# FangjinhuaWang/PatchmatchNet

Measured on AMD Instinct MI355X. Metric: depth-maps/sec at 1600x1200 N=5 src views, higher is better.
Workload: dtype f32

## Files before the change

### include/pmn_hip.h

```cpp
#ifndef PMN_HIP_H
#define PMN_HIP_H

#include <stdint.h>

#ifdef __cplusplus
extern "C" {
#endif

#define PMN_ABI_VERSION 25
#define PMN_MLP_FLOATS 340
#define PMN_MAX_DEPTH 64
#define PMN_MAX_NEIGHBORS 17
#define PMN_MAX_FUSE_SRC 32
#define PMN_TSDF_MAX_VIEWS 16
#define PMN_TSDF_MARK_SPAN 8
#define PMN_RASTER_MAX_DIM 16384
#define PMN_RASTER_MAX_BOX 64
#define PMN_SPLAT_MAX_RADIUS 32

#define PMN_OK 0
#define PMN_ERR_ARG (-1)
#define PMN_ERR_SHAPE (-2)
#define PMN_ERR_LAUNCH (-3)

// ... 36 lines not shown
               int W, int cin, int cout, int K, int stride, int pad, int dil, int relu, int in_nchw, int out_nchw,
               int up_h, int up_w, void *stream);

int pmn_fpn_tail(const float *x, const float *up, const float *w_in, const float *b_in, const float *w_out, float *out,
                 int N, int H, int W, int cin, int cmid, int cout, void *stream);

int pmn_conv2d_mfma(const float *in, const float *weights, const float *shift, float *out, float *out_b, int N, int H, int W,
                    int cin, int cout, int ca, int K, int stride, int pad, int dil, int relu, int planar, void *stream);


int pmn_conv2d_f16s(const float *in, const void *weights, const float *shift, float *out, int N, int H, int W, int cin, int cout,
                    int k, int stride, int relu, void *stream);

int pmn_conv2d_f16s_pair(const float *in, const void *weights_a, const float *shift_a, const void *weights_b, const float *shift_b,
                         float *out, int N, int H, int W, int channels, int relu, void *stream);

int pmn_offset_heads_f16s(const float *in, const void *weights, const float *shift, float *out_a, float *out_b, int N, int H, int W,
                          int cin, int cout, int ca, int dil, void *stream);

int pmn_fpn_level(const float *x, const float *u, const float *w, const float *b, float *out_a, float *out_b, int N, int H,
                  int W, int cin, int cout, int ca, void *stream);

int pmn_deconv3x3s2(const float *in, const float *weights, const float *shift, float *out, int N, int Hi, int Wi, int cin,
                    int cout, int relu, void *stream);

int pmn_refine_front(const float *img, const float *t2, const float *w0, const float *s0, const float *wd, const float *sd,
                     float *x16, int B, int H, int W, void *stream);
int pmn_refine_tail(const float *x16, const float *w3, const float *s3, const float *wr, const float *dnorm,
                    const float *depth_min, const float *depth_max, float *out, int B, int H, int W, void *stream);

int pmn_refine_fused(const float *img, const float *t2, const float *w0, const float *s0, const float *wd, const float *sd,
                     const void *w3a, const float *s3, const float *wr, const float *dnorm, const float *depth_min,
                     const float *depth_max, float *out, int B, int H, int W, void *stream);

int pmn_stage_projections(const float *intrinsics, const float *extrinsics, int B, int V, int nstages, float scale0,
                          float *rel, void *stream);

int pmn_stem(const float *img, const float *w0, const float *s0, const float *w1, const float *s1, float *out, int N, int H,
             int W, void *stream);

int pmn_stem_f16s(const float *img, const float *w0, const float *s0, const void *w1a, const float *s1, float *out, int N, int H,
                  int W, void *stream);

int pmn_stem_f16s_views(const float *const *img_table, int views, const float *w0, const float *s0, const void *w1a,
                        const float *s1, float *out, int B, int H, int W, void *stream);

int pmn_differentiable_warping(const float *src_nchw, const float *rel_proj, const float *depth, int B, int C,
                               int D, int h, int w, int hs, int ws, float *warped, void *stream);

int pmn_fuse_view(const float *maps, long long slot_stride, int ref_slot, const int *src_slots_host,
                  const int *src_hw_host, int n_src, const float *mats, int H, int W, float geo_pixel_thres, float geo_depth_thres, int geo_mask_thres,
                  float photo_thres, unsigned char *masks, float *xyz, double *depth_avg, int *geo_sum, void *stream);

int pmn_fuse_view_merged(const float *maps, long long slot_stride, int ref_slot, const int *src_slots_host,
                         const int *src_hw_host, int n_src, const float *mats, int H, int W, float geo_pixel_thres,
                         float geo_depth_thres, int geo_mask_thres, float photo_thres, unsigned char *masks, float *xyz,
                         double *depth_avg, int *geo_sum, unsigned char *claimed, long long claim_stride, unsigned char *emit,
                         void *stream);

int pmn_pack_points(const unsigned char *final_mask, const float *xyz, const void *image_hwc, int image_is_float, int H, int W,
                    unsigned char *records, long long capacity_points, long long *cursor, int *view_count, long long *scratch,
                    void *stream);

int pmn_pack_points_normals(const unsigned char *final_mask, const float *xyz, const float *normals_chw, const float *rotation,
                            int rotation_stride, const void *image_hwc, int image_is_float, int H, int W, unsigned char *records,
                            long long capacity_points, long long *cursor, int *view_count, long long *scratch, void *stream);
// ... 156 lines not shown
```

### patchmatchnet_amd/_lib.py

```python
from __future__ import annotations

import ctypes
import os
import subprocess
from typing import Optional

_CSRC = os.path.join(os.path.dirname(os.path.abspath(__file__)), "csrc")
LIB_PATH = os.path.join(_CSRC, "libpmn_hip.so")
ABI_VERSION = 25
MLP_FLOATS = 340
MAX_DEPTH = 64
MAX_NEIGHBORS = 17
MAX_FUSE_SRC = 32
TSDF_MAX_VIEWS = 16
TSDF_MARK_SPAN = 8
RASTER_MAX_DIM = 16384
RASTER_MAX_BOX = 64
SPLAT_MAX_RADIUS = 32
ICP_SUMS = 17
ICP_LIMBS = 5
ICP_BLOCK_POINTS = 256
VOXEL_LONG_RUN = 256
VOXEL_MAX_CHANNELS = 8
CROP_MAX_VERTICES = 4096
MESH_PLACE_LONG_RUN = 256
MESH_SIMPLIFY_MAX_FACES = 715827882
MESH_SMOOTH_LONG_ROW = 256
MESH_SMOOTH_MAX_STEPS = 65536
NORMAL_SWEEPS = 6
NORMAL_MAX_VIEWPOINTS = 4096

_fp = ctypes.c_void_p
_ip = ctypes.c_void_p
_hp = ctypes.c_void_p
_i = ctypes.c_int
_f = ctypes.c_float
_s = ctypes.c_void_p

SIGNATURES = {
    "pmn_abi_version": [],
    "pmn_error_string": [_i],
    "pmn_nchw_to_nhwc": [_fp, _fp, _i, _i, _i, _i, _s],
    "pmn_feature_weight": [_fp, _fp, _hp, _fp, _i, _i, _i, _i, _i, _i, _fp, _s],
    "pmn_init_hypotheses": [_fp, _fp, _i, _fp, _fp, _i, _f, _fp, _hp, _i, _i, _i, _i, _fp, _fp, _s],
    "pmn_warp_correlate": [_fp, _fp, _fp, _fp, _fp, _i, _fp, _fp, _i, _i, _i, _i, _i, _i, _i, _i, _i, _fp, _fp, _ip,
                           _fp, _s],
    "pmn_warp_correlate_views": [_fp, _fp, _fp, _fp, _fp, _i, _fp, _fp, _i, _i, _i, _i, _i, _i, _i, _i, _i, _fp, _fp, _ip,
                                 _fp, _s],
    "pmn_aggregate_regress": [_fp, _fp, _fp, _fp, _fp, _hp, _i, _f, _i, _i, _i, _i, _i, _fp, _fp, _s],
    "pmn_confidence": [_fp, _i, _i, _i, _i, _i, _i, _fp, _ip, _s],
    "pmn_conv2d": [_fp, _fp, _fp, _fp, _fp] + [_i] * 14 + [_s],
    "pmn_fpn_tail": [_fp] * 6 + [_i] * 6 + [_s],
    "pmn_fpn_level": [_fp] * 6 + [_i] * 6 + [_s],
    "pmn_conv2d_f16s": [_fp] * 4 + [_i] * 8 + [_s],
    "pmn_offset_heads_f16s": [_fp] * 5 + [_i] * 7 + [_s],
    "pmn_conv2d_f16s_pair": [_fp] * 6 + [_i] * 5 + [_s],
    "pmn_refine_front": [_fp] * 7 + [_i] * 3 + [_s],
    "pmn_refine_tail": [_fp] * 8 + [_i] * 3 + [_s],
    "pmn_refine_fused": [_fp] * 13 + [_i] * 3 + [_s],
    "pmn_conv2d_mfma": [_fp] * 5 + [_i] * 12 + [_s],
    "pmn_deconv3x3s2": [_fp] * 4 + [_i] * 6 + [_s],
    "pmn_stage_projections": [_fp, _fp, _i, _i, _i, _f, _fp, _s],
    "pmn_stem": [_fp] * 6 + [_i] * 3 + [_s],
    "pmn_stem_f16s": [_fp] * 6 + [_i] * 3 + [_s],
    "pmn_stem_f16s_views": [_fp, _i] + [_fp] * 5 + [_i] * 3 + [_s],
    "pmn_differentiable_warping": [_fp, _fp, _fp, _i, _i, _i, _i, _i, _i, _i, _fp, _s],
    "pmn_fuse_view": [_fp, ctypes.c_longlong, _i, _hp, _hp, _i, _fp, _i, _i, _f, _f, _i, _f, _fp, _fp, _fp, _ip, _s],
    "pmn_fuse_view_merged": [_fp, ctypes.c_longlong, _i, _hp, _hp, _i, _fp, _i, _i, _f, _f, _i, _f, _fp, _fp, _fp, _ip, _fp,
                             ctypes.c_longlong, _fp, _s],
    "pmn_pack_points": [_fp, _fp, _fp, _i, _i, _i, _fp, ctypes.c_longlong, _fp, _ip, _fp, _s],
    "pmn_pack_points_normals": [_fp, _fp, _fp, _fp, _i, _fp, _i, _i, _i, _fp, ctypes.c_longlong, _fp, _ip, _fp, _s],
    "pmn_depth_normals": [_fp, _i, _i, _hp, _i, _f, _fp, _s],
    "pmn_normalize_depth": [_fp, _fp, _fp, _i, _i, _fp, _s],
    "pmn_check_f16_domain": [_fp, ctypes.c_longlong, _ip, _s],
    "pmn_plan_create": [ctypes.POINTER(ctypes.c_void_p)],
    "pmn_plan_begin": [_hp],
    "pmn_plan_end": [_hp],
    "pmn_plan_count": [_hp],
    "pmn_plan_kernel_name": [_hp, _i],
    "pmn_plan_launch": [_hp, _s],
    "pmn_plan_destroy": [_hp],
    "pmn_plan_fork": [_hp],
    "pmn_plan_switch": [_hp, _i],
    "pmn_plan_join": [_hp],
    "pmn_plan_entry_branch": [_hp, _i],
    "pmn_plan_launch_part": [_hp, _i, _s],
    "pmn_view_scores": [_fp] * 6 + [_i, _i, ctypes.c_longlong, ctypes.c_longlong] + [ctypes.c_double] * 3 + [_fp, _s],
    "pmn_depth_metrics": [_fp, _fp, _hp, _hp, _hp, _i, _hp, _i, _i, _i, _i, _fp, ctypes.c_longlong, _fp, _s],
    "pmn_nn_distance": [_fp, _ip, ctypes.c_longlong, _hp, ctypes.c_double, _hp, _fp, _ip, ctypes.c_longlong, ctypes.c_double, _fp, _ip,
                        _s],
    "pmn_reduce_round": [_fp, _ip, ctypes.c_longlong, _hp, ctypes.c_double, _hp, ctypes.c_double, _ip, _ip, _ip, _s],
    "pmn_tsdf_integrate": [_fp] * 4 + [_hp, _hp, _f, _f, _fp, ctypes.c_longlong] + [_hp] * 5 + [_i, _s],
# ... 101 lines not shown
```

### patchmatchnet_amd/csrc/misc.hip

```cpp
#include <cstring>

#include "pmn_common.hpp"

extern "C" int pmn_abi_version(void) { return PMN_ABI_VERSION; }

extern "C" const char* pmn_error_string(int code) {
    switch (code) {
        case PMN_OK: return "ok";
        case PMN_ERR_ARG: return "invalid argument (null pointer or size out of range)";
        case PMN_ERR_SHAPE: return "unsupported shape (channels/groups/neighbours/hypotheses)";
        case PMN_ERR_LAUNCH: return "HIP launch failed";
        default: return "unknown error";
    }
}

__global__ __launch_bounds__(PMN_BLOCK) void nchw_to_nhwc_kernel(const float* __restrict__ in, float* __restrict__ out,
                                                                int C, int hw) {
    extern __shared__ float tile[];
    const int b = blockIdx.y, p0 = blockIdx.x * 64, tid = threadIdx.x;
    for (int idx = tid; idx < C * 64; idx += PMN_BLOCK) {
        const int c = idx >> 6, i = idx & 63;
        tile[c * 65 + i] = (p0 + i < hw) ? in[((size_t)b * C + c) * hw + p0 + i] : 0.0f;
    }
    __syncthreads();
// ... 175 lines not shown
            for (int k = 0; k < 4; ++k) acc = acc + P[1][r * 4 + k] * (float)A[k][4 + c];
            o[r * 4 + c] = acc;
        }
}

extern "C" int pmn_stage_projections(const float* intrinsics, const float* extrinsics, int B, int V, int nstages,
                                     float scale0, float* rel, void* stream) {
    if (!intrinsics || !extrinsics || !rel || B < 1 || V < 2 || nstages < 1) return PMN_ERR_ARG;
    const int total = nstages * B * (V - 1);
    PMN_LAUNCH(stage_projections_kernel, dim3((total + 63) / 64), dim3(64), 0, (hipStream_t)stream, intrinsics,
                       extrinsics, B, V, nstages, scale0, rel);
    PMN_CHECK_LAUNCH();
    return PMN_OK;
}

__global__ __launch_bounds__(PMN_BLOCK) void normalize_depth_kernel(const float* __restrict__ depth, const float* __restrict__ depth_min,
                                                                    const float* __restrict__ depth_max, int n, float* __restrict__ out) {
#pragma clang fp contract(off)
    const int b = blockIdx.y, i = blockIdx.x * PMN_BLOCK + threadIdx.x;
    if (i >= n) return;
    const float lo = depth_min[b], span = depth_max[b] - lo;
    out[(size_t)b * n + i] = (depth[(size_t)b * n + i] - lo) / span;
}

extern "C" int pmn_normalize_depth(const float* depth, const float* depth_min, const float* depth_max, int B, int n, float* out,
                                   void* stream) {
    if (!depth || !depth_min || !depth_max || !out || B < 1 || n < 1) return PMN_ERR_ARG;
    PMN_LAUNCH(normalize_depth_kernel, dim3((n + PMN_BLOCK - 1) / PMN_BLOCK, B), dim3(PMN_BLOCK), 0, (hipStream_t)stream, depth,
               depth_min, depth_max, n, out);
    PMN_CHECK_LAUNCH();
    return PMN_OK;
}

__global__ __launch_bounds__(PMN_BLOCK) void check_f16_domain_kernel(const float* __restrict__ x, long long n, int* __restrict__ flag) {
    bool bad = false;
    for (long long i = blockIdx.x * (long long)PMN_BLOCK + threadIdx.x; i < n; i += (long long)gridDim.x * PMN_BLOCK) {
        const float v = fabsf(x[i]);
        bad |= !(v < 65504.0f);
    }
    if (__any(bad) && (threadIdx.x & 63) == 0) atomicOr(flag, 1);
}

extern "C" int pmn_check_f16_domain(const float* x, long long n, int* flag, void* stream) {
    if (!x || !flag || n < 1) return PMN_ERR_ARG;
    const long long blocks = (n + PMN_BLOCK - 1) / PMN_BLOCK;
    PMN_LAUNCH(check_f16_domain_kernel, dim3((unsigned)(blocks < 4096 ? blocks : 4096)), dim3(PMN_BLOCK), 0, (hipStream_t)stream, x, n, flag);
    PMN_CHECK_LAUNCH();
    return PMN_OK;
}
```

### patchmatchnet_amd/csrc/refine.hip

```cpp
#include "conv_common.hpp"

typedef const float __attribute__((address_space(4))) cfloat;

__global__ __launch_bounds__(PMN_BLOCK) void refine_front_kernel(const float* __restrict__ img, const float* __restrict__ t2,
                                                                 const float* __restrict__ w0, const float* __restrict__ s0,
                                                                 const float* __restrict__ wd, const float* __restrict__ sd,
                                                                 float* __restrict__ x16, int B, int H, int W) {
    constexpr int TW = 16, TH = 16, IW = 18, IWP = 19, TP = 9, TPP = 12;
    __shared__ float xin[3 * IW * IWP];
    __shared__ float4 tp4[TP * TP * TPP / 4];
    float* tp = reinterpret_cast<float*>(tp4);
    const cfloat* cw0 = (const cfloat*)w0;
    const cfloat* cs0 = (const cfloat*)s0;
    const cfloat* cwd = (const cfloat*)wd;
    const cfloat* csd = (const cfloat*)sd;
    const int tid = threadIdx.x, wave = __builtin_amdgcn_readfirstlane(tid >> 6), lane = tid & 63;
    const int tiles_x = (W + TW - 1) / TW, tiles_y = (H + TH - 1) / TH;
    const int bt = pmn_xcd_tile(blockIdx.x, B * tiles_x * tiles_y);
    const int n = bt / (tiles_x * tiles_y), tr = bt - n * tiles_x * tiles_y;
    const int oy0 = (tr / tiles_x) * TH, ox0 = (tr % tiles_x) * TW;
    const int Hi = H / 2, Wi = W / 2, iy0 = oy0 / 2, ix0 = ox0 / 2;

    {
        constexpr int NL = (3 * IW * IW + PMN_BLOCK - 1) / PMN_BLOCK;
// ... 158 lines not shown
#pragma unroll
    for (int ky = 0; ky < 3; ++ky)
#pragma unroll
        for (int kx = 0; kx < 3; ++kx) {
            const float* mp = mid + (ty + ky) * MRP + (tx + kx) * MP;
            const float4 a = *reinterpret_cast<const float4*>(mp), b = *reinterpret_cast<const float4*>(mp + 4);
            const cfloat* wq = cwr + (ky * 3 + kx) * 8;
            res = fmaf(a.x, wq[0], res); res = fmaf(a.y, wq[1], res); res = fmaf(a.z, wq[2], res); res = fmaf(a.w, wq[3], res);
            res = fmaf(b.x, wq[4], res); res = fmaf(b.y, wq[5], res); res = fmaf(b.z, wq[6], res); res = fmaf(b.w, wq[7], res);
        }
    const int oy = oy0 + ty, ox = ox0 + tx;
    if (oy >= H || ox >= W) return;
    {
#pragma clang fp contract(off)
        const float lo = dmin[n], span = dmax[n] - lo;
        const float d = dnorm[((size_t)n * (H / 2) + (oy >> 1)) * (W / 2) + (ox >> 1)] + res;
        out[((size_t)n * H + oy) * W + ox] = d * span + lo;
    }
}

extern "C" int pmn_refine_tail(const float* x16, const float* w3, const float* s3, const float* wr, const float* dnorm,
                               const float* depth_min, const float* depth_max, float* out, int B, int H, int W, void* stream) {
    if (!x16 || !w3 || !s3 || !wr || !dnorm || !depth_min || !depth_max || !out || B < 1 || H < 2 || W < 2 || (H & 1) || (W & 1))
        return PMN_ERR_ARG;
    const size_t lds = (size_t)(20 * 424 + 18 * 256) * sizeof(float);
    if (pmn_raise_dynamic_lds(reinterpret_cast<const void*>(refine_tail_kernel), lds) != PMN_OK) return PMN_ERR_LAUNCH;
    const int blocks = B * ((W + 15) / 16) * ((H + 15) / 16);
    PMN_LAUNCH(refine_tail_kernel, dim3(blocks), dim3(PMN_BLOCK), lds, (hipStream_t)stream, x16, w3, s3, wr, dnorm,
                       depth_min, depth_max, out, B, H, W);
    PMN_CHECK_LAUNCH();
    return PMN_OK;
}

template <bool VEC4>
__global__ __launch_bounds__(PMN_BLOCK, 3) void refine_fused_kernel(
    const float* __restrict__ img, const float* __restrict__ t2, const float* __restrict__ w0, const float* __restrict__ s0,
    const float* __restrict__ wd, const float* __restrict__ sd, const f16x8* __restrict__ w3A, const float* __restrict__ s3,
    const float* __restrict__ wr, const float* __restrict__ dnorm, const float* __restrict__ dmin, const float* __restrict__ dmax,
    float* __restrict__ out, int B, int H, int W) {
    constexpr int TW = 16, TH = 16;
    constexpr int IR = 22, IC = 24;
    constexpr int TP = 11, TPP = 12;
    constexpr int XW = 20, XROWP = 26, XPIX = 16;
    constexpr int XPLANE = XW * XROWP * XPIX;
    constexpr int MW = 18, MP = 12, MRP = 256;
    extern __shared__ float4 rf_lds4[];
    _Float16* xh = reinterpret_cast<_Float16*>(rf_lds4);
    float* region = reinterpret_cast<float*>(xh + 2 * XPLANE);
    float* xin = region;
    float* tp = region + 3 * IR * IC;
    float* mid = region;
    const cfloat* cw0 = (const cfloat*)w0;
    const cfloat* cs0 = (const cfloat*)s0;
    const cfloat* cwd = (const cfloat*)wd;
    const cfloat* csd = (const cfloat*)sd;
    const cfloat* cwr = (const cfloat*)wr;
    const int tid = threadIdx.x, wave = __builtin_amdgcn_readfirstlane(tid >> 6), lane = tid & 63, li = lane & 15, kb = lane >> 4;
    const int tiles_x = (W + TW - 1) / TW, tiles_y = (H + TH - 1) / TH;
    const int bt = pmn_xcd_tile(blockIdx.x, B * tiles_x * tiles_y);
    const int n = bt / (tiles_x * tiles_y), tr = bt - n * tiles_x * tiles_y;
    const int oy0 = (tr / tiles_x) * TH, ox0 = (tr % tiles_x) * TW;
    const int Hi = H / 2, Wi = W / 2, iy0 = oy0 / 2 - 1, ix0 = ox0 / 2 - 1;

    {
        float4 u = make_float4(0.f, 0.f, 0.f, 0.f);
        const int upix = tid >> 1, uq = tid & 1;
        const int ur = upix / TP, uc = upix - ur * TP;
        if (upix < TP * TP) {
            const int gy = iy0 + ur, gx = ix0 + uc;
            if ((unsigned)gy < (unsigned)Hi && (unsigned)gx < (unsigned)Wi)
                u = *reinterpret_cast<const float4*>(t2 + (((size_t)n * Hi + gy) * Wi + gx) * 8 + 4 * uq);
        }
        if constexpr (VEC4) {
            float4 v[3];
            const int j = tid & 7, gx = ox0 - 4 + 4 * j;
#pragma unroll
            for (int k = 0; k < 3; ++k) {
                const int R = (tid >> 3) + 32 * k;
                const int c = (R >= IR) + (R >= 2 * IR), r = R - IR * c, gy = oy0 - 3 + r;
                v[k] = make_float4(0.f, 0.f, 0.f, 0.f);
                if (j < 6 && R < 3 * IR && (unsigned)gy < (unsigned)H && (unsigned)gx < (unsigned)W)
                    v[k] = *reinterpret_cast<const float4*>(img + (((size_t)n * 3 + c) * H + gy) * W + gx);
            }
#pragma unroll
            for (int k = 0; k < 3; ++k) {
                const int R = (tid >> 3) + 32 * k;
                if (j < 6 && R < 3 * IR) *reinterpret_cast<float4*>(xin + R * IC + 4 * j) = v[k];
            }
        } else {
            float v[9];
            const int q = tid & 31, gx = ox0 - 4 + q;
#pragma unroll
            for (int k = 0; k < 9; ++k) {
                const int R = (tid >> 5) + 8 * k;
                const int c = (R >= IR) + (R >= 2 * IR), r = R - IR * c, gy = oy0 - 3 + r;
                v[k] = 0.0f;
                if (q < IC && R < 3 * IR && (unsigned)gy < (unsigned)H && (unsigned)gx < (unsigned)W)
                    v[k] = img[(((size_t)n * 3 + c) * H + gy) * W + gx];
            }
#pragma unroll
            for (int k = 0; k < 9; ++k) {
                const int R = (tid >> 5) + 8 * k;
                if (q < IC && R < 3 * IR) xin[R * IC + q] = v[k];
            }
        }
        if (upix < TP * TP) *reinterpret_cast<float4*>(tp + upix * TPP + 4 * uq) = u;
    }
    f16x8 wa[5][2];
#pragma unroll
    for (int ks = 0; ks < 5; ++ks) {
        wa[ks][0] = w3A[(ks * 2 + 0) * 64 + lane];
        wa[ks][1] = w3A[(ks * 2 + 1) * 64 + lane];
    }
    __syncthreads();

// ... 106 lines not shown
                        const int gy = oy0 - 1 + r, gx = ox0 - 1 + q;
                        f32x4_t v = f32x4_t{0.f, 0.f, 0.f, 0.f};
                        if ((unsigned)gy < (unsigned)H && (unsigned)gx < (unsigned)W) {
                            v = f16s_relu(f16s_epilogue(accM[j], accL[j], sh));
                        }
                        *reinterpret_cast<f32x4_t*>(mid + r * MRP + q * MP + 4 * kb) = v;
                    }
                }
            }
        }
    }
    __syncthreads();

    const int tx = tid % TW, ty = tid / TW;
    float res = 0.0f;
#pragma unroll
    for (int ky = 0; ky < 3; ++ky)
#pragma unroll
        for (int kx = 0; kx < 3; ++kx) {
            const float* mp = mid + (ty + ky) * MRP + (tx + kx) * MP;
            const float4 a = *reinterpret_cast<const float4*>(mp), b = *reinterpret_cast<const float4*>(mp + 4);
            const cfloat* wq = cwr + (ky * 3 + kx) * 8;
            res = fmaf(a.x, wq[0], res); res = fmaf(a.y, wq[1], res); res = fmaf(a.z, wq[2], res); res = fmaf(a.w, wq[3], res);
            res = fmaf(b.x, wq[4], res); res = fmaf(b.y, wq[5], res); res = fmaf(b.z, wq[6], res); res = fmaf(b.w, wq[7], res);
        }
    const int oy = oy0 + ty, ox = ox0 + tx;
    if (oy >= H || ox >= W) return;
    {
#pragma clang fp contract(off)
        const float lo = dmin[n], span = dmax[n] - lo;
        const float d = dnorm[((size_t)n * (H / 2) + (oy >> 1)) * (W / 2) + (ox >> 1)] + res;
        out[((size_t)n * H + oy) * W + ox] = d * span + lo;
    }
}

extern "C" int pmn_refine_fused(const float* img, const float* t2, const float* w0, const float* s0, const float* wd, const float* sd,
                            const void* w3a, const float* s3, const float* wr, const float* dnorm, const float* depth_min,
                            const float* depth_max, float* out, int B, int H, int W, void* stream) {
    if (!img || !t2 || !w0 || !s0 || !wd || !sd || !w3a || !s3 || !wr || !dnorm || !depth_min || !depth_max || !out || B < 1 ||
        H < 2 || W < 2 || (H & 1) || (W & 1))
        return PMN_ERR_ARG;
    const size_t lds = (size_t)2 * 20 * 26 * 16 * sizeof(_Float16) + (size_t)18 * 256 * sizeof(float);
    const int blocks = B * ((W + 15) / 16) * ((H + 15) / 16);
    const bool vec4 = W % 4 == 0 && (reinterpret_cast<uintptr_t>(img) & 15) == 0;
    const auto kern = vec4 ? refine_fused_kernel<true> : refine_fused_kernel<false>;
    if (pmn_raise_dynamic_lds(reinterpret_cast<const void*>(kern), lds) != PMN_OK) return PMN_ERR_LAUNCH;
    PMN_LAUNCH(kern, dim3(blocks), dim3(PMN_BLOCK), lds, (hipStream_t)stream, img, t2, w0, s0, wd, sd,
               reinterpret_cast<const f16x8*>(w3a), s3, wr, dnorm, depth_min, depth_max, out, B, H, W);
    PMN_CHECK_LAUNCH();
    return PMN_OK;
}
```

### patchmatchnet_amd/graph.py

```python
from __future__ import annotations

from typing import Dict, List, Optional, Sequence, Tuple

import torch

from ._lib import PmnError


class GraphedForward:

    def __init__(self, model, max_graphs: int = 8, inputs_in_place: bool = False) -> None:
        self.model, self.max_graphs, self.inputs_in_place = model, max_graphs, inputs_in_place
        self.cache: Dict[Tuple, Tuple] = {}
        self.replays = self.captures = self.evictions = 0

    @staticmethod
    def _alias_pattern(images: Sequence[torch.Tensor]) -> Tuple[int, ...]:
        first: Dict[int, int] = {}
        return tuple(first.setdefault(im.data_ptr(), i) for i, im in enumerate(images))

    @classmethod
    def _signature(cls, images: Sequence[torch.Tensor], intrinsics: torch.Tensor, features) -> Tuple:
        feat = None if features is None else tuple(tuple((s, tuple(t.shape)) for s, t in sorted(f.items())) for f in features)
        return (tuple(tuple(i.shape) for i in images), cls._alias_pattern(images), tuple(intrinsics.shape), feat,
                features is not None and cls._table_ok_cached(features))

    _TABLE_OK: Dict[Tuple, bool] = {}

    @classmethod
    def _table_ok_cached(cls, features) -> bool:
        try:
            key = tuple((s, tuple(t.shape), tuple(t.stride()), t.dtype, t.is_cuda) for f in features for s, t in sorted(f.items()))
        except (AttributeError, TypeError):
            return cls._table_ok(features)
        hit = cls._TABLE_OK.get(key)
        if hit is None:
            if len(cls._TABLE_OK) > 64:
                cls._TABLE_OK.clear()
            hit = cls._TABLE_OK[key] = cls._table_ok(features)
        return hit

    def _images_in_place(self, features) -> bool:
        feature = getattr(self.model, "feature", None)
        if not (self.inputs_in_place and features is None and getattr(self.model, "hip_feature_net", False)
                and feature is not None and feature.f16_split):
            return False
        return "conv1_f16s" in feature._packed()

    def _capture(self, images, intrinsics, extrinsics, depth_min, depth_max, features):
        dev = intrinsics.device
        pattern = self._alias_pattern(images)
        in_place = self._images_in_place(features)
        bufs = [torch.empty_like(im) if pattern[i] == i and not (in_place and i) else None for i, im in enumerate(images)]
        static = dict(images=[bufs[pattern[i]] for i in range(len(images))], intrinsics=torch.empty_like(intrinsics),
                      extrinsics=torch.empty_like(extrinsics), depth_min=torch.empty_like(depth_min),
                      depth_max=torch.empty_like(depth_max),
                      noise=torch.empty((images[0].shape[0], 48, images[0].shape[2] // 8, images[0].shape[3] // 8),
                                        dtype=torch.float32, device=dev),
                      features=None, features_nhwc=None)
        if in_place:
            from . import ops
            static["images"] = [bufs[0]] * len(images)
            static["image_bufs"] = bufs
            static["table_all"] = torch.zeros(len(images), dtype=torch.int64, device=dev)
            static["image_table"] = ops.SourceTable(static["table_all"], (len(images),) + tuple(images[0].shape))
            static["table_host"] = []
        if features is not None and self._table_ok(features):
            from . import ops
            B = images[0].shape[0]
            stages = sorted(features[0])
            ref = {s: torch.empty((B,) + tuple(features[0][s].shape[2:]) + (features[0][s].shape[1],), dtype=torch.float32, device=dev)
                   for s in stages}
            static["ref_nhwc"] = ref
            n_src = len(features) - 1
            static["table_all"] = torch.zeros(len(stages) * n_src, dtype=torch.int64, device=dev)
            static["tables"] = {s: ops.SourceTable(static["table_all"][i * n_src:(i + 1) * n_src],
                                                   (n_src, B) + tuple(features[1][s].shape[2:]) + (features[1][s].shape[1],))
                                for i, s in enumerate(stages)}
            static["features"] = [{s: ref[s].permute(0, 3, 1, 2) for s in stages} for _ in range(len(features))]
            static["table_host"] = []
        elif features is not None:
            B = images[0].shape[0]
            stages = sorted(features[0])
            nhwc = {s: torch.empty((len(features) * B,) + tuple(features[0][s].shape[2:]) + (features[0][s].shape[1],),
                                   dtype=torch.float32, device=dev) for s in stages}
            static["features_nhwc"] = nhwc
            static["features"] = [{s: nhwc[s][v * B:(v + 1) * B].permute(0, 3, 1, 2) for s in stages} for v in range(len(features))]
        self._fill(static, images, intrinsics, extrinsics, depth_min, depth_max, features)

        def run():
            return self.model(list(static["images"]), static["intrinsics"], static["extrinsics"], static["depth_min"],
                              static["depth_max"], features=static["features"], features_nhwc=static["features_nhwc"],
                              noise=static["noise"], source_tables=static.get("tables"), ref_nhwc_maps=static.get("ref_nhwc"),
                              image_table=static.get("image_table"))

        rng = torch.cuda.get_rng_state(dev)
        self._draw(static)
        try:
            handle, out = self._record(run, dev)
# ... 20 lines not shown
        try:
            for s in features[0]:
                shapes = {tuple(f[s].shape) for f in features}
                if len(shapes) != 1:
                    return False
                for f in features:
                    t = f[s]
                    if not (t.is_cuda and t.dtype == torch.float32 and t.permute(0, 2, 3, 1).is_contiguous()):
                        return False
            return len(features) >= 2
        except (AttributeError, KeyError, TypeError):
            return False

    @staticmethod
    def _draw(static) -> None:
        torch.rand(size=tuple(static["noise"].shape), out=static["noise"])

    @staticmethod
    def _stage_addresses(static, addrs) -> None:
        ring = static["table_host"]
        k = static["turn"] = (static.get("turn", -1) + 1) % 8
        if k >= len(ring):
            host = torch.empty(static["table_all"].numel(), dtype=torch.int64).pin_memory()
            ring.append([host, host.numpy(), None])
        host, host_np, ev = ring[k]
        if ev is not None:
            ev.synchronize()
        host_np[:] = addrs
        static["table_all"].copy_(host, non_blocking=True)
        ev = torch.cuda.Event()
        ev.record(torch.cuda.current_stream(static["intrinsics"].device))
        ring[k][2] = ev

    @classmethod
    def _fill(cls, static, images, intrinsics, extrinsics, depth_min, depth_max, features) -> None:
        if "image_table" in static:
            from . import ops
            bufs, addrs, held = static["image_bufs"], [], []
            for i, im in enumerate(images):
                if i == 0 or im.device != static["intrinsics"].device or not ops.SourceTable.image_in_place(im):
                    if bufs[i] is None:
                        bufs[i] = torch.empty(tuple(images[0].shape), dtype=torch.float32, device=static["intrinsics"].device)
                    if bufs[i].data_ptr() != im.data_ptr():
                        bufs[i].copy_(im, non_blocking=True)
                    addrs.append(bufs[i].data_ptr())
                else:
                    im.record_stream(torch.cuda.current_stream(im.device))
                    held.append(im)
                    addrs.append(im.data_ptr())
            static["held_images"] = held
            cls._stage_addresses(static, addrs)
        else:
            done = set()
            for dst, src in zip(static["images"], images):
                if dst.data_ptr() not in done and dst.data_ptr() != src.data_ptr():
                    dst.copy_(src, non_blocking=True)
                done.add(dst.data_ptr())
        static["intrinsics"].copy_(intrinsics, non_blocking=True)
        static["extrinsics"].copy_(extrinsics, non_blocking=True)
        static["depth_min"].copy_(depth_min, non_blocking=True)
        static["depth_max"].copy_(depth_max, non_blocking=True)
        if features is not None and "tables" in static:
            for s, t in features[0].items():
                static["features"][0][s].copy_(t, non_blocking=True)
            cls._stage_addresses(static, [features[1 + v][s].data_ptr() for s in sorted(static["tables"]) for v in range(len(features) - 1)])
        elif features is not None:
            for dst, src in zip(static["features"], features):
                for s, t in src.items():
                    dst[s].copy_(t, non_blocking=True)

    def __call__(self, images: List[torch.Tensor], intrinsics: torch.Tensor, extrinsics: torch.Tensor,
                 depth_min: torch.Tensor, depth_max: torch.Tensor, features: Optional[List[Dict[int, torch.Tensor]]] = None):
        if not intrinsics.is_cuda:
            raise PmnError("GraphedForward replays HIP graphs: the inputs must be on a ROCm device")
        h, w = images[0].shape[-2:]
        if h % 8 or w % 8 or any(tuple(i.shape) != tuple(images[0].shape) for i in images):
            depth, confidence, _ = self.model(images, intrinsics, extrinsics, depth_min, depth_max, features=features)
            return depth, confidence
        key = self._signature(images, intrinsics, features)
        entry = self.cache.pop(key, None)
        if entry is None:
            if len(self.cache) >= self.max_graphs:
                self.cache.pop(next(iter(self.cache)))
                self.evictions += 1
# ... 150 lines not shown
```

### patchmatchnet_amd/net.py

```python
from __future__ import annotations

from typing import Dict, List, Optional, Tuple

import warnings

import numpy as np
import torch
import torch.nn as nn
import torch.nn.functional as F

from . import _lib, ops, params
from ._lib import PmnError
from .module import ConvBnReLU
from .patchmatch import PatchMatch


class FeatureNet(nn.Module):

    def __init__(self) -> None:
        super().__init__()
        spec = [(3, 8, 3, 1, 1), (8, 8, 3, 1, 1), (8, 16, 5, 2, 2), (16, 16, 3, 1, 1), (16, 16, 3, 1, 1),
                (16, 32, 5, 2, 2), (32, 32, 3, 1, 1), (32, 32, 3, 1, 1), (32, 64, 5, 2, 2), (64, 64, 3, 1, 1),
                (64, 64, 3, 1, 1)]
        for i, (cin, cout, k, s, p) in enumerate(spec):
# ... 144 lines not shown
        self.research = dict(layers=False)

    def _packed(self):
        srcs = [p for p in self.parameters()] + [b for b in self.buffers() if b.dtype.is_floating_point]
        key = params.versions(srcs)
        if getattr(self, "_pack_key", None) != key:
            dev = self.res.weight.device

            def bn_of(m):
                return (m.weight, m.bias, m.running_mean, m.running_var)

            pk = {}
            for name in ("conv0", "conv1", "conv2", "conv3"):
                m = getattr(self, name)
                w, s = params.pack_conv(m.conv.weight, bn=bn_of(m.bn), eps=m.bn.eps)
                pk[name] = (torch.from_numpy(w).to(dev), torch.from_numpy(s).to(dev))
            w, s = params.pack_deconv(self.deconv.weight, bn=bn_of(self.bn), eps=self.bn.eps)
            pk["deconv"] = (torch.from_numpy(w).to(dev), torch.from_numpy(s).to(dev))
            w, s = params.pack_conv(self.res.weight)
            pk["res"] = (torch.from_numpy(w).to(dev), torch.from_numpy(s).to(dev))
            pk["tail"] = tuple(torch.from_numpy(a).to(dev) for a in params.pack_refine_tail(
                self.conv3.conv.weight, bn_of(self.conv3.bn), self.res.weight, eps=self.conv3.bn.eps))
            self.f16_domain_error = None
            try:
                w, s = params.pack_refine_conv3_f16s(self.conv3.conv.weight, bn_of(self.conv3.bn), eps=self.conv3.bn.eps)
                pk["conv3_f16s"] = (torch.from_numpy(w).to(dev), torch.from_numpy(s).to(dev))
            except params.F16DomainError as e:
                self.f16_domain_error = f"conv3: {e}"
                warnings.warn("Refinement: " + self.f16_domain_error + " -- using the fp32 kernels (pmn_refine_front / pmn_refine_tail)",
                              RuntimeWarning, stacklevel=2)
            self._pack, self._pack_key = pk, key
        return self._pack

    def forward_hip(self, img: torch.Tensor, depth_0: torch.Tensor, depth_min: torch.Tensor, depth_max: torch.Tensor
                    ) -> torch.Tensor:
        pk = self._packed()
        b = depth_min.size()[0]
        if not self.research["layers"]:
            d = ops.normalize_depth(depth_0, depth_min, depth_max)
        else:
            lo = depth_min.view(b, 1, 1, 1)
            span = (depth_max - depth_min).view(b, 1, 1, 1)
            d = ((depth_0 - lo) / span).contiguous()
        t = ops.conv2d(d, *pk["conv1"], 8, 3, 1, 1, relu=True, in_nchw=True)
        t = ops.conv2d(t, *pk["conv2"], 8, 3, 1, 1, relu=True)
        if not self.research["layers"]:
            if self.f16_split and "conv3_f16s" in pk:
                return ops.refine_fused(img.contiguous(), t, *pk["conv0"], *pk["deconv"], *pk["conv3_f16s"], pk["tail"][2], d,
                                        depth_min.float().contiguous(), depth_max.float().contiguous())
            x16 = ops.refine_front(img.contiguous(), t, *pk["conv0"], *pk["deconv"])
            return ops.refine_tail(x16, *pk["tail"], d, depth_min.float().contiguous(), depth_max.float().contiguous())
        img_feat = ops.conv2d(img.contiguous(), *pk["conv0"], 8, 3, 1, 1, relu=True, in_nchw=True)
        up = ops.deconv3x3s2(t, *pk["deconv"], relu=True)
        t = ops.conv2d(torch.cat((up, img_feat), dim=3), *pk["conv3"], 8, 3, 1, 1, relu=True)
        res = ops.conv2d(t, *pk["res"], 1, 3, 1, 1, out_nchw=True)
        d = F.interpolate(d, scale_factor=2.0, mode="nearest") + res
        return d * span + lo

    def forward(self, img: torch.Tensor, depth_0: torch.Tensor, depth_min: torch.Tensor, depth_max: torch.Tensor
                ) -> torch.Tensor:
        b = depth_min.size()[0]
        lo = depth_min.view(b, 1, 1, 1)
        span = (depth_max - depth_min).view(b, 1, 1, 1)
        d = (depth_0 - lo) / span
        img_feat = self.conv0(img)
        up = F.relu(self.bn(self.deconv(self.conv2(self.conv1(d)))), inplace=True)
        res = self.res(self.conv3(torch.cat((up, img_feat), dim=1)))
        d = F.interpolate(d, scale_factor=2.0, mode="nearest") + res
        return d * span + lo


class PatchmatchNet(nn.Module):

    def __init__(self, patchmatch_interval_scale: List[float], propagation_range: List[int],
                 patchmatch_iteration: List[int], patchmatch_num_sample: List[int], propagate_neighbors: List[int],
                 evaluate_neighbors: List[int]) -> None:
        super().__init__()
        self.stages = 4
        self.feature = FeatureNet()
# ... 123 lines not shown
        for stage in range(self.stages - 1, 0, -1):
            if stage == self.stages - 2:
                ops.plan_join()
                pending.clear()
            if rel_all is None:
                intrinsics_l = intrinsics.clone()
                intrinsics_l[:, :, :2] *= scale
                proj = extrinsics.clone()
                proj[:, :, :3, :4] = torch.matmul(intrinsics_l, extrinsics[:, :, :3, :4])
                proj_l = torch.unbind(proj, 1)
                ref_proj, src_proj = proj_l[0], proj_l[1:]
            else:
                ref_proj, src_proj = extrinsics[:, 0], [extrinsics[:, i] for i in range(1, extrinsics.shape[1])]
            scale *= 2.0

            dbg = [] if debug is not None else None
            pm: PatchMatch = getattr(self, f"patchmatch_{stage}")
            ref_nhwc, src_nhwc = stage_maps(stage)
            depths, score, view_weights = pm(
                ref_feature=ref_feature[stage], src_features=[f[stage] for f in src_features], ref_proj=ref_proj,
                src_projs=list(src_proj), depth_min=depth_min, depth_max=depth_max, depth=depth,
                view_weights=view_weights, depth_shift=depth_shift, vw_shift=vw_shift,
                noise=noise if stage == self.stages - 1 else None, debug=dbg, ref_nhwc=ref_nhwc, src_nhwc=src_nhwc,
                rel_proj=None if rel_all is None else rel_all[self.stages - 1 - stage], precomputed=precomputed.get(stage))
            if debug is not None:
                debug[stage] = dbg
            depth_patchmatch[stage] = depths
            depth = depths[-1].detach()
            if stage > 1:
                depth_shift = 1
                vw_shift = vw_shift + 1 if view_weights.shape[-1] != depths[-1].shape[-1] else 1

        if self.hip_feature_net and ref_image.is_cuda:
            depth = self.upsample_net.forward_hip(ref_image, depth, depth_min, depth_max)
        else:
            depth = self.upsample_net(ref_image, depth, depth_min, depth_max)
        if ref_width != orig_width or ref_height != orig_height:
            depth = F.interpolate(depth, size=[orig_height, orig_width], mode="bilinear", align_corners=False)
        depth_patchmatch[0] = [depth]

        confidence, _ = ops.confidence(score.contiguous(), orig_height, orig_width)
        return depth, confidence, depth_patchmatch


def adjust_image_dims(images: List[torch.Tensor], intrinsics: torch.Tensor
                      ) -> Tuple[List[torch.Tensor], torch.Tensor, int, int]:
    _, _, ref_height, ref_width = images[0].size()
    for i in range(len(images)):
        _, _, height, width = images[i].size()
        new_height = int(round(height / 8)) * 8
        new_width = int(round(width / 8)) * 8
        if new_width != width or new_height != height:
            intrinsics[:, i, 0] *= new_width / width
            intrinsics[:, i, 1] *= new_height / height
            images[i] = F.interpolate(images[i], size=[new_height, new_width], mode="bilinear", align_corners=False)
    return images, intrinsics, ref_height, ref_width
```

### patchmatchnet_amd/ops.py

```python
from __future__ import annotations

import ctypes
import threading
from typing import List, Optional, Sequence, Tuple

import numpy as np
import torch

from . import _lib
from ._lib import PmnError, check


_TIMING = None
_TIMING_ON = True


def enable_kernel_timing() -> None:
    global _TIMING, _TIMING_ON
    _TIMING, _TIMING_ON = [], True


def pause_kernel_timing(paused: bool) -> None:
    global _TIMING_ON
    _TIMING_ON = not paused
# ... 711 lines not shown
        _dev(t_, n_)
    B, H, W, c = x16.shape
    if c != 16 or H % 2 or W % 2 or tuple(dnorm.shape) != (B, 1, H // 2, W // 2) or tuple(w3.shape) != (2, 3, 3, 16, 4) or \
            tuple(wr.shape) != (3, 3, 8) or depth_min.numel() != B or depth_max.numel() != B:
        raise PmnError("refine_tail: inconsistent shapes")
    out = torch.empty((B, 1, H, W), dtype=torch.float32, device=x16.device)
    with torch.cuda.device(x16.device):
        check(_lib.lib().pmn_refine_tail(x16.data_ptr(), w3.data_ptr(), s3.data_ptr(), wr.data_ptr(), dnorm.data_ptr(),
                                         depth_min.data_ptr(), depth_max.data_ptr(), out.data_ptr(), B, H, W, _stream(x16)),
              "pmn_refine_tail")
    return out


def refine_fused(img: torch.Tensor, t2: torch.Tensor, w0: torch.Tensor, s0: torch.Tensor, wd: torch.Tensor, sd: torch.Tensor,
                 w3a: torch.Tensor, s3: torch.Tensor, wr: torch.Tensor, dnorm: torch.Tensor, depth_min: torch.Tensor,
                 depth_max: torch.Tensor) -> torch.Tensor:
    for n_, t_ in (("img", img), ("t2", t2), ("w0", w0), ("s0", s0), ("wd", wd), ("sd", sd), ("s3", s3), ("wr", wr), ("dnorm", dnorm),
                   ("depth_min", depth_min), ("depth_max", depth_max)):
        _dev(t_, n_)
    if tuple(_dev_as(w3a, "refine_fused: w3a", torch.float16).shape) != (5, 2, 64, 8):
        raise PmnError("refine_fused: w3a must be the float16 [5,2,64,8] tensor of params.pack_refine_conv3_f16s")
    B, c, H, W = img.shape
    if c != 3 or H % 2 or W % 2 or tuple(t2.shape) != (B, H // 2, W // 2, 8) or tuple(dnorm.shape) != (B, 1, H // 2, W // 2) or \
            tuple(w0.shape) != (3, 3, 3, 8) or tuple(wd.shape) != (3, 3, 8, 8) or tuple(wr.shape) != (3, 3, 8) or s3.numel() != 8 or \
            depth_min.numel() != B or depth_max.numel() != B:
        raise PmnError("refine_fused: inconsistent shapes")
    _f16_domain_probe(img, t2)
    out = torch.empty((B, 1, H, W), dtype=torch.float32, device=img.device)
    with torch.cuda.device(img.device):
        check(_lib.lib().pmn_refine_fused(img.data_ptr(), t2.data_ptr(), w0.data_ptr(), s0.data_ptr(), wd.data_ptr(), sd.data_ptr(),
                                          w3a.data_ptr(), s3.data_ptr(), wr.data_ptr(), dnorm.data_ptr(), depth_min.data_ptr(),
                                          depth_max.data_ptr(), out.data_ptr(), B, H, W, _stream(img)), "pmn_refine_fused")
    return out


def deconv3x3s2(x: torch.Tensor, weights: torch.Tensor, shift: torch.Tensor, relu: bool = True) -> torch.Tensor:
    _dev(x, "x")
    _dev(weights, "weights")
    _dev(shift, "shift")
    N, Hi, Wi, cin = x.shape
    cout = weights.shape[3]
    out = torch.empty((N, 2 * Hi, 2 * Wi, cout), dtype=torch.float32, device=x.device)
    with torch.cuda.device(x.device):
        check(_lib.lib().pmn_deconv3x3s2(x.data_ptr(), weights.data_ptr(), shift.data_ptr(), out.data_ptr(), N, Hi, Wi, cin,
                                         cout, 1 if relu else 0, _stream(x)), "pmn_deconv3x3s2")
    return out


def stem(img: torch.Tensor, w0: torch.Tensor, s0: torch.Tensor, w1: torch.Tensor, s1: torch.Tensor,
         out: Optional[torch.Tensor] = None) -> torch.Tensor:
    for n_, t_ in (("img", img), ("w0", w0), ("s0", s0), ("w1", w1), ("s1", s1)):
        _dev(t_, n_)
    N, c, H, W = img.shape
    if c != 3 or tuple(w0.shape) != (3, 3, 3, 8) or tuple(w1.shape) != (3, 3, 8, 8):
        raise PmnError("stem: expects a 3-channel image and 3->8->8 weights")
    if out is None:
        out = torch.empty((N, H, W, 8), dtype=torch.float32, device=img.device)
    else:
        _dev(out, "out")
        if tuple(out.shape) != (N, H, W, 8):
            raise PmnError("stem: bad `out` shape")
    with torch.cuda.device(img.device):
        check(_lib.lib().pmn_stem(img.data_ptr(), w0.data_ptr(), s0.data_ptr(), w1.data_ptr(), s1.data_ptr(), out.data_ptr(),
                                  N, H, W, _stream(img)), "pmn_stem")
    return out

# ... 718 lines not shown
```

Baseline: 401.1.

## Read reference image via address table in refine and batch input staging

The fused refinement kernel can now read the reference image through a device-side address table instead of a copied static buffer. This lets graph replay skip copying the reference image into the captured buffer. Staging of the image addresses and the small intrinsics, extrinsics and depth-range copies is merged into one single-block kernel launch, replacing several separate copies. The cost is an extra pointer indirection in the kernel and extra capture-time complexity around aliasing.

Result: no change. 402.7 (median of 6 runs) (+0.4%).

```diff
diff --git a/include/pmn_hip.h b/include/pmn_hip.h
--- a/include/pmn_hip.h
+++ b/include/pmn_hip.h
@@ -92,6 +92,17 @@
 int pmn_refine_fused(const float *img, const float *t2, const float *w0, const float *s0, const float *wd, const float *sd,
                      const void *w3a, const float *s3, const float *wr, const float *dnorm, const float *depth_min,
                      const float *depth_max, float *out, int B, int H, int W, void *stream);
+
+int pmn_refine_fused_table(const float *const *img_table, int entry, const float *t2, const float *w0, const float *s0,
+                           const float *wd, const float *sd, const void *w3a, const float *s3, const float *wr,
+                           const float *dnorm, const float *depth_min, const float *depth_max, float *out, int B, int H, int W,
+                           void *stream);
+
+#define PMN_STAGE_MAX_IMAGES 16
+int pmn_stage_inputs(const void *const *image_addrs_host, int n_images, void **table, const float *intrinsics,
+                     float *intrinsics_out, int n_intrinsics, const float *extrinsics, float *extrinsics_out, int n_extrinsics,
+                     const float *depth_min, float *depth_min_out, int n_depth_min, const float *depth_max, float *depth_max_out,
+                     int n_depth_max, void *stream);
 
 int pmn_stage_projections(const float *intrinsics, const float *extrinsics, int B, int V, int nstages, float scale0,
                           float *rel, void *stream);
diff --git a/patchmatchnet_amd/_lib.py b/patchmatchnet_amd/_lib.py
--- a/patchmatchnet_amd/_lib.py
+++ b/patchmatchnet_amd/_lib.py
@@ -12,6 +12,7 @@
 MAX_DEPTH = 64
 MAX_NEIGHBORS = 17
 MAX_FUSE_SRC = 32
+STAGE_MAX_IMAGES = 16
 TSDF_MAX_VIEWS = 16
 TSDF_MARK_SPAN = 8
 RASTER_MAX_DIM = 16384
@@ -58,6 +59,8 @@
     "pmn_refine_front": [_fp] * 7 + [_i] * 3 + [_s],
     "pmn_refine_tail": [_fp] * 8 + [_i] * 3 + [_s],
     "pmn_refine_fused": [_fp] * 13 + [_i] * 3 + [_s],
+    "pmn_refine_fused_table": [_fp, _i] + [_fp] * 12 + [_i] * 3 + [_s],
+    "pmn_stage_inputs": [_hp, _i, _fp] + [_fp, _fp, _i] * 4 + [_s],
     "pmn_conv2d_mfma": [_fp] * 5 + [_i] * 12 + [_s],
     "pmn_deconv3x3s2": [_fp] * 4 + [_i] * 6 + [_s],
     "pmn_stage_projections": [_fp, _fp, _i, _i, _i, _f, _fp, _s],
diff --git a/patchmatchnet_amd/csrc/misc.hip b/patchmatchnet_amd/csrc/misc.hip
--- a/patchmatchnet_amd/csrc/misc.hip
+++ b/patchmatchnet_amd/csrc/misc.hip
@@ -231,6 +231,59 @@
     return PMN_OK;
 }
 
+struct StageInputsArgs {
+    unsigned long long addr[PMN_STAGE_MAX_IMAGES];
+    unsigned long long* table;
+    const float* src[4];
+    float* dst[4];
+    int count[4];
+    int n_images;
+};
+
+__global__ __launch_bounds__(PMN_BLOCK) void stage_inputs_kernel(const StageInputsArgs a) {
+    const int tid = threadIdx.x;
+    unsigned long long mine = 0;
+#pragma unroll
+    for (int k = 0; k < PMN_STAGE_MAX_IMAGES; ++k) mine = tid == k ? a.addr[k] : mine;
+    if (tid < a.n_images) a.table[tid] = mine;
+#pragma unroll
+    for (int k = 0; k < 4; ++k) {
+        const float* __restrict__ s = a.src[k];
+        float* __restrict__ d = a.dst[k];
+        for (int i = tid; i < a.count[k]; i += PMN_BLOCK) d[i] = s[i];
+    }
+}
+
+extern "C" int pmn_stage_inputs(const void* const* image_addrs_host, int n_images, void** table, const float* intrinsics,
+                                float* intrinsics_out, int n_intrinsics, const float* extrinsics, float* extrinsics_out,
+                                int n_extrinsics, const float* depth_min, float* depth_min_out, int n_depth_min,
+                                const float* depth_max, float* depth_max_out, int n_depth_max, void* stream) {
+    if (n_images < 0 || n_images > PMN_STAGE_MAX_IMAGES || (n_images > 0 && (!image_addrs_host || !table))) return PMN_ERR_ARG;
+    StageInputsArgs a;
+    memset(&a, 0, sizeof(a));
+    for (int k = 0; k < n_images; ++k) {
+        if (!image_addrs_host[k]) return PMN_ERR_ARG;
+        a.addr[k] = (unsigned long long)reinterpret_cast<uintptr_t>(image_addrs_host[k]);
+    }
+    a.table = reinterpret_cast<unsigned long long*>(table);
+    a.n_images = n_images;
+    const float* src[4] = {intrinsics, extrinsics, depth_min, depth_max};
+    float* dst[4] = {intrinsics_out, extrinsics_out, depth_min_out, depth_max_out};
+    const int count[4] = {n_intrinsics, n_extrinsics, n_depth_min, n_depth_max};
+    bool any = n_images > 0;
+    for (int k = 0; k < 4; ++k) {
+        if (count[k] < 0 || (count[k] > 0 && (!src[k] || !dst[k]))) return PMN_ERR_ARG;
+        a.src[k] = src[k];
+        a.dst[k] = dst[k];
+        a.count[k] = count[k];
+        any = any || count[k] > 0;
+    }
+    if (!any) return PMN_ERR_ARG;
+    PMN_LAUNCH(stage_inputs_kernel, dim3(1), dim3(PMN_BLOCK), 0, (hipStream_t)stream, a);
+    PMN_CHECK_LAUNCH();
+    return PMN_OK;
+}
+
 __global__ __launch_bounds__(PMN_BLOCK) void check_f16_domain_kernel(const float* __restrict__ x, long long n, int* __restrict__ flag) {
     bool bad = false;
     for (long long i = blockIdx.x * (long long)PMN_BLOCK + threadIdx.x; i < n; i += (long long)gridDim.x * PMN_BLOCK) {
diff --git a/patchmatchnet_amd/csrc/refine.hip b/patchmatchnet_amd/csrc/refine.hip
--- a/patchmatchnet_amd/csrc/refine.hip
+++ b/patchmatchnet_amd/csrc/refine.hip
@@ -214,9 +214,17 @@
     return PMN_OK;
 }
 
-template <bool VEC4>
-__global__ __launch_bounds__(PMN_BLOCK, 3) void refine_fused_kernel(
-    const float* __restrict__ img, const float* __restrict__ t2, const float* __restrict__ w0, const float* __restrict__ s0,
+typedef const float __attribute__((address_space(1))) * rf_gfloat;
+typedef float rf_f4n __attribute__((ext_vector_type(4)));
+__device__ __forceinline__ float4 rf_load4(const float* p) { return *reinterpret_cast<const float4*>(p); }
+__device__ __forceinline__ float4 rf_load4(rf_gfloat p) {
+    const rf_f4n v = *(const rf_f4n __attribute__((address_space(1)))*)p;
+    return make_float4(v.x, v.y, v.z, v.w);
+}
+
+template <bool VEC4, typename ImgPtr>
+__device__ __forceinline__ void refine_fused_body(
+    const ImgPtr img, const float* __restrict__ t2, const float* __restrict__ w0, const float* __restrict__ s0,
     const float* __restrict__ wd, const float* __restrict__ sd, const f16x8* __restrict__ w3A, const float* __restrict__ s3,
     const float* __restrict__ wr, const float* __restrict__ dnorm, const float* __restrict__ dmin, const float* __restrict__ dmax,
     float* __restrict__ out, int B, int H, int W) {
@@ -262,7 +270,7 @@
                 const int c = (R >= IR) + (R >= 2 * IR), r = R - IR * c, gy = oy0 - 3 + r;
                 v[k] = make_float4(0.f, 0.f, 0.f, 0.f);
                 if (j < 6 && R < 3 * IR && (unsigned)gy < (unsigned)H && (unsigned)gx < (unsigned)W)
-                    v[k] = *reinterpret_cast<const float4*>(img + (((size_t)n * 3 + c) * H + gy) * W + gx);
+                    v[k] = rf_load4(img + (((size_t)n * 3 + c) * H + gy) * W + gx);
             }
 #pragma unroll
             for (int k = 0; k < 3; ++k) {
@@ -435,6 +443,25 @@
         const float d = dnorm[((size_t)n * (H / 2) + (oy >> 1)) * (W / 2) + (ox >> 1)] + res;
         out[((size_t)n * H + oy) * W + ox] = d * span + lo;
     }
+}
+
+template <bool VEC4>
+__global__ __launch_bounds__(PMN_BLOCK, 3) void refine_fused_kernel(
+    const float* __restrict__ img, const float* __restrict__ t2, const float* __restrict__ w0, const float* __restrict__ s0,
+    const float* __restrict__ wd, const float* __restrict__ sd, const f16x8* __restrict__ w3A, const float* __restrict__ s3,
+    const float* __restrict__ wr, const float* __restrict__ dnorm, const float* __restrict__ dmin, const float* __restrict__ dmax,
+    float* __restrict__ out, int B, int H, int W) {
+    refine_fused_body<VEC4, const float* __restrict__>(img, t2, w0, s0, wd, sd, w3A, s3, wr, dnorm, dmin, dmax, out, B, H, W);
+}
+
+template <bool VEC4>
+__global__ __launch_bounds__(PMN_BLOCK, 3) void refine_fused_kernel_tab(
+    const float* const* __restrict__ img_slot, const float* __restrict__ t2, const float* __restrict__ w0,
+    const float* __restrict__ s0, const float* __restrict__ wd, const float* __restrict__ sd, const f16x8* __restrict__ w3A,
+    const float* __restrict__ s3, const float* __restrict__ wr, const float* __restrict__ dnorm, const float* __restrict__ dmin,
+    const float* __restrict__ dmax, float* __restrict__ out, int B, int H, int W) {
+    const rf_gfloat img = (rf_gfloat)*img_slot;
+    refine_fused_body<VEC4, rf_gfloat>(img, t2, w0, s0, wd, sd, w3A, s3, wr, dnorm, dmin, dmax, out, B, H, W);
 }
 
 extern "C" int pmn_refine_fused(const float* img, const float* t2, const float* w0, const float* s0, const float* wd, const float* sd,
@@ -453,3 +480,20 @@
     PMN_CHECK_LAUNCH();
     return PMN_OK;
 }
+
+extern "C" int pmn_refine_fused_table(const float* const* img_table, int entry, const float* t2, const float* w0, const float* s0,
+                                      const float* wd, const float* sd, const void* w3a, const float* s3, const float* wr,
+                                      const float* dnorm, const float* depth_min, const float* depth_max, float* out, int B, int H,
+                                      int W, void* stream) {
+    if (!img_table || entry < 0 || !t2 || !w0 || !s0 || !wd || !sd || !w3a || !s3 || !wr || !dnorm || !depth_min || !depth_max ||
+        !out || B < 1 || H < 2 || W < 2 || (H & 1) || (W & 1))
+        return PMN_ERR_ARG;
+    const size_t lds = (size_t)2 * 20 * 26 * 16 * sizeof(_Float16) + (size_t)18 * 256 * sizeof(float);
+    const int blocks = B * ((W + 15) / 16) * ((H + 15) / 16);
+    const auto kern = W % 4 == 0 ? refine_fused_kernel_tab<true> : refine_fused_kernel_tab<false>;
+    if (pmn_raise_dynamic_lds(reinterpret_cast<const void*>(kern), lds) != PMN_OK) return PMN_ERR_LAUNCH;
+    PMN_LAUNCH(kern, dim3(blocks), dim3(PMN_BLOCK), lds, (hipStream_t)stream, img_table + entry, t2, w0, s0, wd, sd,
+               reinterpret_cast<const f16x8*>(w3a), s3, wr, dnorm, depth_min, depth_max, out, B, H, W);
+    PMN_CHECK_LAUNCH();
+    return PMN_OK;
+}
diff --git a/patchmatchnet_amd/graph.py b/patchmatchnet_amd/graph.py
--- a/patchmatchnet_amd/graph.py
+++ b/patchmatchnet_amd/graph.py
@@ -47,10 +47,15 @@
             return False
         return "conv1_f16s" in feature._packed()
 
+    def _reference_in_place(self) -> bool:
+        refine = getattr(self.model, "upsample_net", None)
+        return refine is not None and hasattr(refine, "reads_table") and refine.reads_table()
+
     def _capture(self, images, intrinsics, extrinsics, depth_min, depth_max, features):
         dev = intrinsics.device
         pattern = self._alias_pattern(images)
         in_place = self._images_in_place(features)
+        ref_in_place = in_place and self._reference_in_place()
         bufs = [torch.empty_like(im) if pattern[i] == i and not (in_place and i) else None for i, im in enumerate(images)]
         static = dict(images=[bufs[pattern[i]] for i in range(len(images))], intrinsics=torch.empty_like(intrinsics),
                       extrinsics=torch.empty_like(extrinsics), depth_min=torch.empty_like(depth_min),
@@ -62,9 +67,9 @@
             from . import ops
             static["images"] = [bufs[0]] * len(images)
             static["image_bufs"] = bufs
+            static["ref_in_place"] = ref_in_place
             static["table_all"] = torch.zeros(len(images), dtype=torch.int64, device=dev)
             static["image_table"] = ops.SourceTable(static["table_all"], (len(images),) + tuple(images[0].shape))
-            static["table_host"] = []
         if features is not None and self._table_ok(features):
             from . import ops
             B = images[0].shape[0]
@@ -151,13 +156,28 @@
         ev.record(torch.cuda.current_stream(static["intrinsics"].device))
         ring[k][2] = ev
 
+    @staticmethod
+    def _stage_inputs(static, addrs, intrinsics, extrinsics, depth_min, depth_max) -> None:
+        from . import ops
+        pairs = []
+        for name, src in (("intrinsics", intrinsics), ("extrinsics", extrinsics), ("depth_min", depth_min), ("depth_max", depth_max)):
+            dst = static[name]
+            if src.device == dst.device and src.dtype == torch.float32 and src.shape == dst.shape and src.is_contiguous() and \
+                    dst.is_contiguous() and src.data_ptr() != dst.data_ptr():
+                pairs.append((src, dst))
+            else:
+                dst.copy_(src, non_blocking=True)
+                pairs.append((None, dst))
+        ops.stage_inputs(static["table_all"], addrs, pairs)
+
     @classmethod
     def _fill(cls, static, images, intrinsics, extrinsics, depth_min, depth_max, features) -> None:
         if "image_table" in static:
             from . import ops
             bufs, addrs, held = static["image_bufs"], [], []
             for i, im in enumerate(images):
-                if i == 0 or im.device != static["intrinsics"].device or not ops.SourceTable.image_in_place(im):
+                if (i == 0 and not static["ref_in_place"]) or im.device != static["intrinsics"].device or \
+                        not ops.SourceTable.image_in_place(im):
                     if bufs[i] is None:
                         bufs[i] = torch.empty(tuple(images[0].shape), dtype=torch.float32, device=static["intrinsics"].device)
                     if bufs[i].data_ptr() != im.data_ptr():
@@ -168,7 +188,8 @@
                     held.append(im)
                     addrs.append(im.data_ptr())
             static["held_images"] = held
-            cls._stage_addresses(static, addrs)
+            cls._stage_inputs(static, addrs, intrinsics, extrinsics, depth_min, depth_max)
+            return
         else:
             done = set()
             for dst, src in zip(static["images"], images):
diff --git a/patchmatchnet_amd/net.py b/patchmatchnet_amd/net.py
--- a/patchmatchnet_amd/net.py
+++ b/patchmatchnet_amd/net.py
@@ -200,8 +200,11 @@
             self._pack, self._pack_key = pk, key
         return self._pack
 
-    def forward_hip(self, img: torch.Tensor, depth_0: torch.Tensor, depth_min: torch.Tensor, depth_max: torch.Tensor
-                    ) -> torch.Tensor:
+    def reads_table(self) -> bool:
+        return bool(self.f16_split and not self.research["layers"] and "conv3_f16s" in self._packed())
+
+    def forward_hip(self, img: torch.Tensor, depth_0: torch.Tensor, depth_min: torch.Tensor, depth_max: torch.Tensor,
+                    image_table: Optional["ops.SourceTable"] = None) -> torch.Tensor:
         pk = self._packed()
         b = depth_min.size()[0]
         if not self.research["layers"]:
@@ -213,6 +216,9 @@
         t = ops.conv2d(d, *pk["conv1"], 8, 3, 1, 1, relu=True, in_nchw=True)
         t = ops.conv2d(t, *pk["conv2"], 8, 3, 1, 1, relu=True)
         if not self.research["layers"]:
+            if image_table is not None and self.reads_table():
+                return ops.refine_fused_table(image_table, 0, t, *pk["conv0"], *pk["deconv"], *pk["conv3_f16s"], pk["tail"][2], d,
+                                              depth_min.float().contiguous(), depth_max.float().contiguous())
             if self.f16_split and "conv3_f16s" in pk:
                 return ops.refine_fused(img.contiguous(), t, *pk["conv0"], *pk["deconv"], *pk["conv3_f16s"], pk["tail"][2], d,
                                         depth_min.float().contiguous(), depth_max.float().contiguous())
@@ -402,7 +408,7 @@
                 vw_shift = vw_shift + 1 if view_weights.shape[-1] != depths[-1].shape[-1] else 1
 
         if self.hip_feature_net and ref_image.is_cuda:
-            depth = self.upsample_net.forward_hip(ref_image, depth, depth_min, depth_max)
+            depth = self.upsample_net.forward_hip(ref_image, depth, depth_min, depth_max, image_table=image_table)
         else:
             depth = self.upsample_net(ref_image, depth, depth_min, depth_max)
         if ref_width != orig_width or ref_height != orig_height:
diff --git a/patchmatchnet_amd/ops.py b/patchmatchnet_amd/ops.py
--- a/patchmatchnet_amd/ops.py
+++ b/patchmatchnet_amd/ops.py
@@ -767,6 +767,54 @@
                                           w3a.data_ptr(), s3.data_ptr(), wr.data_ptr(), dnorm.data_ptr(), depth_min.data_ptr(),
                                           depth_max.data_ptr(), out.data_ptr(), B, H, W, _stream(img)), "pmn_refine_fused")
     return out
+
+
+def refine_fused_table(images: "SourceTable", entry: int, t2: torch.Tensor, w0: torch.Tensor, s0: torch.Tensor, wd: torch.Tensor,
+                       sd: torch.Tensor, w3a: torch.Tensor, s3: torch.Tensor, wr: torch.Tensor, dnorm: torch.Tensor,
+                       depth_min: torch.Tensor, depth_max: torch.Tensor) -> torch.Tensor:
+    for n_, t_ in (("t2", t2), ("w0", w0), ("s0", s0), ("wd", wd), ("sd", sd), ("s3", s3), ("wr", wr), ("dnorm", dnorm),
+                   ("depth_min", depth_min), ("depth_max", depth_max)):
+        _dev(t_, n_)
+    if not isinstance(images, SourceTable) or len(images.shape) != 5 or images.shape[2] != 3 or not 0 <= int(entry) < images.shape[0]:
+        raise PmnError("refine_fused_table: a SourceTable of shape (views, B, 3, H, W) and an entry inside it")
+    if tuple(_dev_as(w3a, "refine_fused_table: w3a", torch.float16).shape) != (5, 2, 64, 8):
+        raise PmnError("refine_fused_table: w3a must be the float16 [5,2,64,8] tensor of params.pack_refine_conv3_f16s")
+    _, B, _, H, W = images.shape
+    if H % 2 or W % 2 or tuple(t2.shape) != (B, H // 2, W // 2, 8) or tuple(dnorm.shape) != (B, 1, H // 2, W // 2) or \
+            tuple(w0.shape) != (3, 3, 3, 8) or tuple(wd.shape) != (3, 3, 8, 8) or tuple(wr.shape) != (3, 3, 8) or s3.numel() != 8 or \
+            depth_min.numel() != B or depth_max.numel() != B:
+        raise PmnError("refine_fused_table: inconsistent shapes")
+    _f16_domain_probe(t2)
+    out = torch.empty((B, 1, H, W), dtype=torch.float32, device=images.device)
+    with torch.cuda.device(images.device):
+        check(_lib.lib().pmn_refine_fused_table(images.table.data_ptr(), int(entry), t2.data_ptr(), w0.data_ptr(), s0.data_ptr(),
+                                                wd.data_ptr(), sd.data_ptr(), w3a.data_ptr(), s3.data_ptr(), wr.data_ptr(),
+                                                dnorm.data_ptr(), depth_min.data_ptr(), depth_max.data_ptr(), out.data_ptr(), B, H, W,
+                                                _stream(out)), "pmn_refine_fused_table")
+    return out
+
+
+def stage_inputs(table: Optional[torch.Tensor], addresses: Sequence[int], pairs: Sequence[Tuple[Optional[torch.Tensor], torch.Tensor]]
+                 ) -> None:
+    if len(pairs) != 4 or len(addresses) > _lib.STAGE_MAX_IMAGES:
+        raise PmnError(f"stage_inputs: four (source, destination) pairs and at most {_lib.STAGE_MAX_IMAGES} addresses")
+    dev = (table if table is not None else pairs[0][1]).device
+    args = []
+    for src, dst in pairs:
+        if src is None:
+            args += [None, None, 0]
+            continue
+        if _dev(src, "stage_inputs: source").numel() != _dev(dst, "stage_inputs: destination").numel() or src.device != dev or \
+                dst.device != dev:
+            raise PmnError("stage_inputs: a source and its destination hold the same number of floats, on one device")
+        args += [src.data_ptr(), dst.data_ptr(), src.numel()]
+    n = len(addresses)
+    if n and (table is None or table.dtype != torch.int64 or table.device != dev or not table.is_contiguous() or table.numel() < n):
+        raise PmnError("stage_inputs: the table is a dense int64 device tensor with room for every address")
+    host = (ctypes.c_void_p * n)(*addresses) if n else None
+    with torch.cuda.device(dev):
+        check(_lib.lib().pmn_stage_inputs(host, n, table.data_ptr() if n else None, *args,
+                                          torch.cuda.current_stream(dev).cuda_stream), "pmn_stage_inputs")
 
 
 def deconv3x3s2(x: torch.Tensor, weights: torch.Tensor, shift: torch.Tensor, relu: bool = True) -> torch.Tensor:
```
